# SimMarkt/RL_PtG

Measured on AMD Instinct MI355X. Metric: env-steps/sec at N=65536 envs; achieved HBM GB/s vs roofline, higher is better.
Workload: dtype f32 observations / rewards; env state, reward coefficients and cum_rew in f64

## Files before the change

### rl_ptg_amd/csrc/ptg_env.hip

```cpp
#include "ptg_handle.h"

#include <hip/hip_runtime.h>
#include <chrono>
#include <hip/hip_ext.h>

#include <algorithm>
#include <cmath>
#include <cstdarg>
#include <cstdio>
#include <cstdlib>
#include <cstring>
#include <string>
#include <type_traits>
#include <vector>

namespace {

constexpr int NT = PTG_N_TABLES;
constexpr int NC = PTG_N_COLS;
constexpr int N_DEST = 6;
constexpr int DEST_TID[N_DEST] = {PTG_T_COOLDOWN, PTG_T_STANDBY_UP, PTG_T_STANDBY_DOWN, PTG_T_STARTUP_COLD,
                                  PTG_T_STARTUP_HOT, PTG_T_OP1_START_P};

__device__ __forceinline__ int part_tid(int p) { return p == 0 ? PTG_T_OP1_START_P : 7 + p; }
// ... 2104 lines not shown
        if (std::chrono::steady_clock::now() - t0 > std::chrono::microseconds(200)) break;
    }
    HIP_TRY(h, hipStreamSynchronize(st));
    return 0;
}

int collect_error(ptg_env* h, hipStream_t st)
{
    const int rc = wait_stream(h, st);
    if (rc) return rc;
    return check_error_flags(h);
}

struct FinSpan { unsigned s0, n, c0, dropped; };
__device__ __forceinline__ FinSpan fin_span(unsigned total, unsigned ring_cap, unsigned cap, const unsigned* count, int append)
{
    FinSpan s;
    const unsigned have = total < ring_cap ? total : ring_cap;
    const unsigned held = append ? count[0] : 0u;
    s.c0 = held < cap ? held : cap;
    const unsigned room = cap - s.c0;
    s.n = have < room ? have : room;
    s.s0 = (total - have) % ring_cap;
    s.dropped = total - s.n;
    return s;
}

__global__ void __launch_bounds__(256)
k_fin_drain(const double* __restrict__ r_ret, const int* __restrict__ r_len, const int* __restrict__ r_env, const unsigned* __restrict__ r_count,
            unsigned ring_cap, double* __restrict__ ret, int* __restrict__ len, int* __restrict__ env, unsigned cap,
            const unsigned* __restrict__ count, int append, int env_offset)
{
    const FinSpan s = fin_span(*r_count, ring_cap, cap, count, append);
    for (unsigned i = blockIdx.x * 256u + threadIdx.x; i < s.n; i += gridDim.x * 256u) {
        unsigned slot = s.s0 + i;
        if (slot >= ring_cap) slot -= ring_cap;
        if (ret) ret[s.c0 + i] = r_ret[slot];
        if (len) len[s.c0 + i] = r_len[slot];
        if (env) env[s.c0 + i] = r_env[slot] + env_offset;
    }
}

__global__ void __launch_bounds__(64)
k_fin_commit(unsigned* r_count, unsigned ring_cap, unsigned cap, unsigned* count, int append)
{
    if (threadIdx.x != 0) return;
    const FinSpan s = fin_span(*r_count, ring_cap, cap, count, append);
    const unsigned before = append ? count[1] : 0u;
    count[0] = s.c0 + s.n;
    count[1] = before + s.dropped;
    *r_count = 0u;
}

__global__ void __launch_bounds__(1024)
k_fin_stats(const double* __restrict__ ret, const int* __restrict__ len, const unsigned* __restrict__ count, double* __restrict__ stats,
            int accumulate)
{
    __shared__ double part[16][5];
    const unsigned n = count[0];
    double s = 0.0, s2 = 0.0, sl = 0.0, mn = INFINITY, mx = -INFINITY;
#pragma unroll 4
    for (unsigned i = threadIdx.x; i < n; i += 1024u) {
        const double r = ret[i];
        s += r; s2 += r * r;
        if (len) sl += (double)len[i];
        mn = r < mn ? r : mn; mx = r > mx ? r : mx;
    }
    for (int off = 32; off > 0; off >>= 1) {
        s += __shfl_down(s, off); s2 += __shfl_down(s2, off); sl += __shfl_down(sl, off);
        const double a = __shfl_down(mn, off), b = __shfl_down(mx, off);
        mn = a < mn ? a : mn; mx = b > mx ? b : mx;
    }
    const int wave = threadIdx.x >> 6;
    if ((threadIdx.x & 63) == 0) { part[wave][0] = s; part[wave][1] = s2; part[wave][2] = sl; part[wave][3] = mn; part[wave][4] = mx; }
    __syncthreads();
    if (threadIdx.x != 0) return;
    for (int w = 1; w < 16; w++) {
        s += part[w][0]; s2 += part[w][1]; sl += part[w][2];
        mn = part[w][3] < mn ? part[w][3] : mn; mx = part[w][4] > mx ? part[w][4] : mx;
    }
    double c = (double)n;
    if (accumulate) {
        c += stats[0]; s += stats[1]; s2 += stats[2]; sl += stats[3];
        mn = stats[4] < mn ? stats[4] : mn; mx = stats[5] > mx ? stats[5] : mx;
    }
    stats[0] = c; stats[1] = s; stats[2] = s2; stats[3] = sl; stats[4] = mn; stats[5] = mx;
}

}

extern "C" {

int ptg_abi_version(void) { return PTG_ABI_VERSION; }

const char* ptg_last_error(const ptg_env* env) { return env ? env->err.c_str() : g_create_err.c_str(); }

int ptg_num_envs(const ptg_env* env) { return env ? env->n : PTG_E_INVALID; }
int ptg_obs_dim(const ptg_env* env) { return env ? env->F : PTG_E_INVALID; }

void ptg_destroy(ptg_env* env)
{
    if (!env) return;
    (void)hipSetDevice(env->device);
    (void)hipDeviceSynchronize();
    if (env->ref_stream) (void)hipStreamDestroy(env->ref_stream);
    if (env->ev_fork) (void)hipEventDestroy(env->ev_fork);
    if (env->ev_tail) (void)hipEventDestroy(env->ev_tail);
    for (void* p : env->allocs) (void)hipFree(p);
    if (env->d_tape) (void)hipFree(env->d_tape);
    if (env->d_eps_ind) (void)hipFree(env->d_eps_ind);
    if (env->vn_partials) (void)hipFree(env->vn_partials);
    if (env->vn_den) (void)hipFree(env->vn_den);
    if (env->vn_moments) (void)hipFree(env->vn_moments);
    if (env->err_host) (void)hipHostFree(env->err_host);
    if (env->fin_stage) (void)hipHostFree(env->fin_stage);
    for (void* q : {env->hs_act, env->hs_out, env->hs_final, (void*)env->hs_info}) if (q) (void)hipFree(q);
    for (auto& r : env->prof_used)
        for (hipEvent_t e : {r.e0, r.e1, r.h0, r.h1}) if (e) (void)hipEventDestroy(e);
    for (auto& p : env->prof_free) { (void)hipEventDestroy(p.first); (void)hipEventDestroy(p.second); }
    delete env;
}

int ptg_create(const ptg_config* cfg, const ptg_tables* tables, const ptg_market* sets, int n_sets, int n_envs,
               int device_id, ptg_env** out)
{
    if (!cfg || !tables || !sets || !out) return set_err(nullptr, PTG_E_INVALID, "ptg_create: null argument");
    if (n_envs <= 0 || n_sets < 1 || n_sets > PTG_MAX_MARKET_SETS) return set_err(nullptr, PTG_E_INVALID, "ptg_create: bad n_envs / n_sets");
    if (cfg->time_step_op <= 0 || cfg->sim_step <= 0 || cfg->price_ahead < 1 || cfg->price_ahead > 64)
        return set_err(nullptr, PTG_E_INVALID, "ptg_create: bad sim_step / time_step_op / price_ahead");
    if (cfg->out_dtype != PTG_OUT_F32 && cfg->out_dtype != PTG_OUT_F64) return set_err(nullptr, PTG_E_INVALID, "ptg_create: bad out_dtype");
    if (cfg->obs_layout < PTG_OBS_ROW_MAJOR || cfg->obs_layout > PTG_OBS_SPLIT) return set_err(nullptr, PTG_E_INVALID, "ptg_create: bad obs_layout");
    if (cfg->eps_sim_steps < 7) return set_err(nullptr, PTG_E_INVALID, "ptg_create: eps_sim_steps must be >= 7");
    int ndev = 0;
    hipError_t he = hipGetDeviceCount(&ndev);
    if (he != hipSuccess || ndev <= 0)
        return set_err(nullptr, PTG_E_HIP, "no HIP device available (%s): libptg_env has no CPU path", hipGetErrorString(he));
    if (device_id < 0 || device_id >= ndev) return set_err(nullptr, PTG_E_INVALID, "device %d out of range (%d devices)", device_id, ndev);
    he = hipSetDevice(device_id);
    if (he != hipSuccess) return set_err(nullptr, PTG_E_HIP, "hipSetDevice failed: %s", hipGetErrorString(he));

    ptg_env* h = new ptg_env();
    h->cfg = *cfg; h->n = n_envs; h->device = device_id; h->n_sets = n_sets;
    h->knob_no_hot = getenv("PTG_NO_HOT_KERNELS") != nullptr; h->knob_no_lds_lut = getenv("PTG_NO_LDS_LUT") != nullptr;
    h->knob_no_refresh = getenv("PTG_NO_REFRESH") != nullptr; h->knob_refresh_always = getenv("PTG_REFRESH_ALWAYS") != nullptr;
    {
        hipDeviceProp_t prop;
        if (hipGetDeviceProperties(&prop, device_id) == hipSuccess && prop.multiProcessorCount > 0) h->n_cu = prop.multiProcessorCount;
        else (void)hipGetLastError();
    }
    if (const char* v = getenv("PTG_PC_CHUNK")) h->knob_chunk = atoi(v);
    if (const char* v = getenv("PTG_BLOCK")) { const int b = atoi(v); if (b == 128 || b == 256 || b == 512) h->knob_block = b; }
    h->S = (int)((double)cfg->sim_step / (double)cfg->time_step_op);
    h->F = cfg->raw_modified ? 2 * cfg->price_ahead + 9 : cfg->price_ahead + 4 + 9;
    h->fast = (cfg->out_dtype == PTG_OUT_F32);
    h->fm = (cfg->obs_layout == PTG_OBS_FEATURE_MAJOR);
    memset(&h->P, 0, sizeof h->P);
    DevParams& P = h->P;
    int rc = 0;
    auto fail = [&](int code) { g_create_err = h->err; ptg_destroy(h); return code; };
    if (h->S < 1) { set_err(h, PTG_E_INVALID, "step_size < 1"); return fail(PTG_E_INVALID); }
// ... 72 lines not shown
        float2* d_sc32;
        if ((rc = dev_upload(h, &d_sc32, sc32.data(), sc32.size()))) return fail(rc);
        P.sincos32 = d_sc32;
        std::vector<float>& pool = h->pool32_host;
        h->off_sc = (unsigned)pool.size();
        for (size_t q = 0; q < sc32.size(); q++) { pool.push_back(sc32[q].x); pool.push_back(sc32[q].y); }
        pool.resize(pool.size() + 16, 0.f);
        float* d_pool;
        if ((rc = dev_upload(h, &d_pool, pool.data(), pool.size()))) return fail(rc);
        h->d_pool32 = d_pool;
        P.featA32 = d_pool; P.featB32 = d_pool + h->off_featB; P.gas_n32 = d_pool + h->off_gasn; P.eua_n32 = d_pool + h->off_euan;
        pool.clear(); pool.shrink_to_fit();
        std::vector<double>& p64 = h->pool64_host;
        h->o64_sc = (unsigned)p64.size();
        for (size_t q = 0; q < sc.size(); q++) { p64.push_back(sc[q].x); p64.push_back(sc[q].y); }
        p64.resize(p64.size() + 16, 0.0);
        double* d_p64;
        if ((rc = dev_upload(h, &d_p64, p64.data(), p64.size()))) return fail(rc);
        h->d_pool64 = d_p64;
        p64.clear(); p64.shrink_to_fit();
    }
    {
        const double f = P.sim_step_d / 3600;
        P.k_chp = cfg->convert_mol_to_Nm3 * cfg->H_u_CH4 * 1000 * (cfg->eta_CHP * cfg->eeg_el_price + (1 - cfg->eta_CHP) * cfg->heat_price) * f;
        P.k_eua = cfg->Molar_mass_CO2 / 1000 / 1000 * 3600 * 100 * f;
        RecFast* d_recf;
        if ((rc = dev_alloc(h, &d_recf, h->rec_total))) return fail(rc);
        hipLaunchKernelGGL(k_build_fast, dim3(grid_for((long long)h->rec_total, 256)), dim3(256), 0, 0, P, P.rec, d_recf, (int)h->rec_total);
        if ((rc = launch_check(h, "k_build_fast"))) return fail(rc);
        P.recf = d_recf;
        if ((rc = dev_alloc(h, &h->d_rkey, h->rec_total + 8))) return fail(rc);
        hipLaunchKernelGGL(k_extract_keys, dim3(grid_for((long long)h->rec_total, 256)), dim3(256), 0, 0, d_recf, h->d_rkey, (int)h->rec_total);
        if ((rc = launch_check(h, "k_extract_keys"))) return fail(rc);
    }

    if ((rc = dev_alloc(h, &P.st_a, n_envs)) || (rc = dev_alloc(h, &P.st_b, n_envs)) || (rc = dev_alloc(h, &P.st_c, n_envs)))
        return fail(rc);
    P.fin_cap = std::max(2 * n_envs, 1024);
    if ((rc = dev_alloc(h, &P.fin_ret, P.fin_cap)) || (rc = dev_alloc(h, &P.fin_len, P.fin_cap)) ||
        (rc = dev_alloc(h, &P.fin_env, P.fin_cap)) || (rc = dev_alloc(h, &P.fin_count, 1)))
        return fail(rc);
    {
        void* dp = nullptr;
        if (hipHostMalloc((void**)&h->err_host, 6 * sizeof(int), hipHostMallocMapped) != hipSuccess ||
            hipHostGetDevicePointer(&dp, h->err_host, 0) != hipSuccess) { set_err(h, PTG_E_HIP, "hipHostMalloc of the error words failed"); return fail(PTG_E_HIP); }
        h->err_host[0] = 0; h->err_host[1] = 0; h->err_host[2] = 0; h->err_host[3] = 0; h->err_host[4] = 0; h->err_host[5] = 0;
        P.err = (int*)dp;
    }
    if ((rc = dev_alloc(h, &P.term_flag, 4))) return fail(rc);
    if (hipMemset(P.term_flag, 0, 4 * sizeof(int)) != hipSuccess) { set_err(h, PTG_E_HIP, "hipMemset failed"); return fail(PTG_E_HIP); }
    h->d_desync = P.term_flag + 1;
    if ((rc = set_desync(h, nullptr, true, true))) return fail(rc);
    {
        const size_t need = (size_t)P.fin_cap * (sizeof(double) + 2 * sizeof(int));
        if (hipHostMalloc(&h->fin_stage, need, hipHostMallocDefault) == hipSuccess) h->fin_stage_bytes = need;
        else { (void)hipGetLastError(); h->fin_stage = nullptr; }
    }
    if (hipMemset(P.fin_count, 0, sizeof(int)) != hipSuccess) {
        set_err(h, PTG_E_HIP, "hipMemset failed");
        return fail(PTG_E_HIP);
    }
    {
        const int lad[LAD_N] = {P.t1_start_p_f, P.t2_start_f_p, P.t_p_f, P.t_f_p, P.t1_p_f_p, P.t2_p_f_p, P.t3_p_f_p, P.t34_p_f_p, P.t4_p_f_p,
                                P.t45_p_f_p, P.t5_p_f_p, P.t1_f_p_f, P.t2_f_p_f, P.t23_f_p_f, P.t3_f_p_f, P.t34_f_p_f, P.t4_f_p_f, P.t45_f_p_f,
                                P.t5_f_p_f, P.i_full, P.j_full};
        if ((rc = dev_upload(h, &h->d_ladder, lad, LAD_N))) return fail(rc);
    }
    hipLaunchKernelGGL(k_init_state, dim3(grid_for(n_envs, 256)), dim3(256), 0, 0, P, 0, 0);
    if ((rc = launch_check(h, "k_init_state"))) return fail(rc);
    if (!h->knob_no_refresh) {
        int lo = 0, hi = 0;
        (void)hipDeviceGetStreamPriorityRange(&lo, &hi);
        if (hipStreamCreateWithPriority(&h->ref_stream, hipStreamNonBlocking, hi) != hipSuccess) { h->ref_stream = nullptr; (void)hipGetLastError(); }
        if (hipEventCreateWithFlags(&h->ev_fork, hipEventDisableTiming) != hipSuccess) {
            (void)hipGetLastError();
            if (h->ref_stream) { (void)hipStreamDestroy(h->ref_stream); h->ref_stream = nullptr; }
        }
    }
    if (hipDeviceSynchronize() != hipSuccess) { set_err(h, PTG_E_HIP, "device synchronize failed after init"); return fail(PTG_E_HIP); }
    *out = h;
    return 0;
}

int ptg_set_market_assignment(ptg_env* h, const uint8_t* set_of_env_host)
{
    if (!h || !set_of_env_host) return set_err(h, PTG_E_INVALID, "null argument");
    HIP_TRY(h, hipSetDevice(h->device));
    HIP_TRY(h, hipDeviceSynchronize());
    std::vector<StA> a(h->n);
    HIP_TRY(h, hipMemcpy(a.data(), h->P.st_a, sizeof(StA) * h->n, hipMemcpyDeviceToHost));
    for (int e = 0; e < h->n; e++) {
        if (set_of_env_host[e] >= h->n_sets) return set_err(h, PTG_E_INVALID, "env %d: market set %d out of range", e, set_of_env_host[e]);
        a[e].flags = (a[e].flags & ~(3u << 15)) | ((unsigned)set_of_env_host[e] << 15);
    }
    HIP_TRY(h, hipMemcpy(h->P.st_a, a.data(), sizeof(StA) * h->n, hipMemcpyHostToDevice));
    return 0;
}

int ptg_set_episode_plan(ptg_env* h, const double* eps_ind_host, int n, int64_t first_ptr, int64_t stride)
{
    if (!h || n < 0 || (n > 0 && !eps_ind_host) || first_ptr < 0 || stride < 0) return set_err(h, PTG_E_INVALID, "bad episode plan");
    HIP_TRY(h, hipSetDevice(h->device));
    if (h->d_eps_ind) { (void)hipFree(h->d_eps_ind); h->d_eps_ind = nullptr; }
    h->P.E = n; h->P.eps_ind = nullptr; h->P.ep_stride = 0;
    if (n > 0) {
        std::vector<int> ei(n);
        for (int q = 0; q < n; q++) ei[q] = (int)eps_ind_host[q];
        HIP_TRY(h, hipMalloc((void**)&h->d_eps_ind, sizeof(int) * n));
        HIP_TRY(h, hipMemcpy(h->d_eps_ind, ei.data(), sizeof(int) * n, hipMemcpyHostToDevice));
        h->P.eps_ind = h->d_eps_ind;
        h->P.ep_stride = (int)(stride % n);
    }
    hipLaunchKernelGGL(k_init_state, dim3(grid_for(h->n, 256)), dim3(256), 0, 0, h->P, n > 0 ? (int)(first_ptr % n) : 0, 1);
    int rc = launch_check(h, "k_init_state");
// ... 83 lines not shown
    return 0;
}

int ptg_set_global_env_offset(ptg_env* h, int64_t offset)
{
    if (!h || offset < 0) return set_err(h, PTG_E_INVALID, "bad env offset");
    h->P.env_offset = (long long)offset;
    return 0;
}

int ptg_get_noise_tape(ptg_env* h, double* tape_host)
{
    if (!h || !tape_host) return set_err(h, PTG_E_INVALID, "null argument");
    if (h->tape_len <= 0) return set_err(h, PTG_E_INVALID, "no noise tape set");
    HIP_TRY(h, hipSetDevice(h->device));
    HIP_TRY(h, hipDeviceSynchronize());
    double* tmp = nullptr;
    const size_t bytes = sizeof(double) * (size_t)h->n * h->tape_len;
    HIP_TRY(h, hipMalloc((void**)&tmp, bytes));
    hipLaunchKernelGGL(k_transpose, dim3((h->n + 31) / 32, (h->tape_len + 31) / 32), dim3(32, 8), 0, 0, (const double*)h->d_tape, tmp, h->tape_len, h->n);
    hipError_t e = hipDeviceSynchronize();
    if (e == hipSuccess) e = hipMemcpy(tape_host, tmp, bytes, hipMemcpyDeviceToHost);
    (void)hipFree(tmp);
    if (e != hipSuccess) return set_err(h, PTG_E_HIP, "noise tape download failed: %s", hipGetErrorString(e));
    return 0;
}

int ptg_reset(ptg_env* h, const uint8_t* mask_host, void* obs_dev, void* stream)
{
    if (!h) return PTG_E_INVALID;
    HIP_TRY(h, hipSetDevice(h->device));
    hipStream_t st = as_stream(stream);
    uint8_t* d_mask = nullptr;
    if (mask_host) {
        HIP_TRY(h, hipMalloc((void**)&d_mask, h->n));
        HIP_TRY(h, hipMemcpyAsync(d_mask, mask_host, h->n, hipMemcpyHostToDevice, st));
    }
    const dim3 grid(grid_for(h->n, 256)), block(256);
    if (h->cfg.out_dtype == PTG_OUT_F64) {
        if (h->fm) hipLaunchKernelGGL((k_reset<double, false, true, 0>), grid, block, 0, st, h->P, d_mask, (double*)obs_dev);
        else hipLaunchKernelGGL((k_reset<double, false, false, 0>), grid, block, 0, st, h->P, d_mask, (double*)obs_dev);
    } else {
        if (h->fm) hipLaunchKernelGGL((k_reset<float, true, true, 0>), grid, block, 0, st, h->P, d_mask, (float*)obs_dev);
        else hipLaunchKernelGGL((k_reset<float, true, false, 0>), grid, block, 0, st, h->P, d_mask, (float*)obs_dev);
    }
    int rc = launch_check(h, "k_reset");
    if (d_mask) { (void)hipStreamSynchronize(st); (void)hipFree(d_mask); }
    if (rc) return rc;
    bool all = !mask_host;
    if (mask_host) { all = true; for (int e = 0; e < h->n && all; e++) all = mask_host[e] != 0; }
    if (all) { h->reset_done = true; h->sync_k = 0; }
    else h->sync_k = -1;
    return set_desync(h, st, !all);
}

static int launch_step_generic(ptg_env* h, hipStream_t st, const void* actions_dev, int action_kind, void* obs_dev, void* rew_dev,
                               uint8_t* done_dev, void* final_obs_dev, double* info_dev, int only_at_k = -1)
{
    const dim3 grid(grid_for(h->n, 256)), block(256);
    const bool f64 = h->cfg.out_dtype == PTG_OUT_F64;
    h->fin_maybe = true;
#define PTG_LAUNCH_STEP_(OUT, FAST, INFO, FM, PAC)                                                                     \
    hipLaunchKernelGGL((k_step<OUT, FAST, INFO, FM, PAC>), grid, block, 0, st, h->P, actions_dev, action_kind, (OUT*)obs_dev, \
                       (OUT*)rew_dev, done_dev, (OUT*)final_obs_dev, info_dev, only_at_k)
#define PTG_LAUNCH_STEP(OUT, FAST, INFO, FM)                                                                          \
    do { if (h->cfg.price_ahead == 13) PTG_LAUNCH_STEP_(OUT, FAST, INFO, FM, 13); else PTG_LAUNCH_STEP_(OUT, FAST, INFO, FM, 0); } while (0)
    if (f64) {
        if (info_dev) { if (h->fm) PTG_LAUNCH_STEP(double, false, true, true); else PTG_LAUNCH_STEP(double, false, true, false); }
        else { if (h->fm) PTG_LAUNCH_STEP(double, false, false, true); else PTG_LAUNCH_STEP(double, false, false, false); }
    } else if (info_dev) {
        if (h->fm) PTG_LAUNCH_STEP(float, false, true, true); else PTG_LAUNCH_STEP(float, false, true, false);
    } else {
        if (h->fm) PTG_LAUNCH_STEP(float, true, false, true); else PTG_LAUNCH_STEP(float, true, false, false);
    }
#undef PTG_LAUNCH_STEP
#undef PTG_LAUNCH_STEP_
    return launch_check(h, "k_step");
}

static int launch_rollout_generic(ptg_env* h, hipStream_t st, const void* actions_dev, int action_kind, int n_steps, void* obs_dev,
                                  void* rew_dev, uint8_t* done_dev, double* info_dev = nullptr)
{
    const size_t asz = action_kind == PTG_ACT_I64 ? 8 : 4, osz = h->cfg.out_dtype == PTG_OUT_F64 ? 8 : 4;
    for (int t = 0; t < n_steps; t++) {
        const int rc = launch_step_generic(h, st, (const char*)actions_dev + (size_t)t * h->n * asz, action_kind,
                                           (char*)obs_dev + (size_t)t * obs_step_elems(h) * osz, (char*)rew_dev + (size_t)t * h->n * osz,
                                           done_dev + (size_t)t * h->n, nullptr, info_dev ? info_dev + (size_t)t * h->n * PTG_N_INFO : nullptr);
        if (rc) return rc;
    }
    return 0;
}

int ptg_step(ptg_env* h, const void* actions_dev, int action_kind, void* obs_dev, void* rew_dev, uint8_t* done_dev,
             void* final_obs_dev, double* info_dev, void* stream)
{
    if (!h) return PTG_E_INVALID;
    if (!actions_dev || !obs_dev || !rew_dev || !done_dev) return set_err(h, PTG_E_INVALID, "ptg_step: null buffer");
    if (action_kind < PTG_ACT_I32 || action_kind > PTG_ACT_I64) return set_err(h, PTG_E_INVALID, "ptg_step: bad action_kind");
    if ((h->cfg.action_type == 1) != (action_kind == PTG_ACT_F32))
        return set_err(h, PTG_E_INVALID, "ptg_step: action_kind does not match cfg.action_type");
    if (!h->reset_done) return set_err(h, PTG_E_INVALID, "ptg_step: envs must be reset first");
    HIP_TRY(h, hipSetDevice(h->device));
    hipStream_t st = as_stream(stream);
    const int k_term = h->cfg.eps_sim_steps - 6;
    if (hot_eligible(h) && !info_dev && h->sync_k != k_term) {
        hipStreamCaptureStatus cs = hipStreamCaptureStatusNone;
        if (hipStreamIsCapturing(st, &cs) != hipSuccess) { (void)hipGetLastError(); cs = hipStreamCaptureStatusNone; }
        const bool capturing = cs != hipStreamCaptureStatusNone && h->replay_proof;
        h->step_skip_term = capturing ? 1 : 0;
        PTG_HOT_DISPATCH(launch_step_hot, h, st, actions_dev, action_kind, PTG_NOARG, obs_dev, rew_dev, done_dev);
        h->step_skip_term = 0;
        int rc = launch_check(h, "k_step_hot");
        if (!rc && capturing) rc = launch_step_generic(h, st, actions_dev, action_kind, obs_dev, rew_dev, done_dev, final_obs_dev, nullptr, k_term);
        h->sync_k += 1;
        return rc;
    }
    const int rc = launch_step_generic(h, st, actions_dev, action_kind, obs_dev, rew_dev, done_dev, final_obs_dev, info_dev);
    if (h->sync_k >= 0) h->sync_k = (h->sync_k == k_term) ? 0 : h->sync_k + 1;
    return rc;
}

static int rollout_impl(ptg_env* h, const char* what, const void* actions_dev, int action_kind, int n_steps, void* obs_dev, void* rew_dev,
                        uint8_t* done_dev, double* info_dev, void* stream)
{
    if (!h) return PTG_E_INVALID;
    if (!actions_dev || !obs_dev || !rew_dev || !done_dev || n_steps < 1) return set_err(h, PTG_E_INVALID, "%s: bad argument", what);
    if (action_kind < PTG_ACT_I32 || action_kind > PTG_ACT_I64) return set_err(h, PTG_E_INVALID, "%s: bad action_kind", what);
    if ((h->cfg.action_type == 1) != (action_kind == PTG_ACT_F32))
        return set_err(h, PTG_E_INVALID, "%s: action_kind does not match cfg.action_type", what);
    if (!h->reset_done) return set_err(h, PTG_E_INVALID, "%s: envs must be reset first", what);
// ... 18 lines not shown
            rc = launch_check(h, "k_rollout_pc");
            h->sync_k += cnt;
        } else if (h->sync_k >= 0) {
            cnt = 1;
            rc = launch_rollout_generic(h, st, a_t, action_kind, 1, o_t, r_t, d_t, i_t);
            h->sync_k = (h->sync_k == k_term) ? 0 : h->sync_k + 1;
        } else {
            cnt = n_steps - t0;
            rc = launch_rollout_generic(h, st, a_t, action_kind, cnt, o_t, r_t, d_t, i_t);
        }
        if (rc) return rc;
        t0 += cnt;
    }
    return 0;
}

int ptg_rollout(ptg_env* h, const void* actions_dev, int action_kind, int n_steps, void* obs_dev, void* rew_dev,
                uint8_t* done_dev, void* stream)
{
    return rollout_impl(h, "ptg_rollout", actions_dev, action_kind, n_steps, obs_dev, rew_dev, done_dev, nullptr, stream);
}

int ptg_rollout_info(ptg_env* h, const void* actions_dev, int action_kind, int n_steps, void* obs_dev, void* rew_dev,
                     uint8_t* done_dev, double* info_dev, void* stream)
{
    if (h && !info_dev) return set_err(h, PTG_E_INVALID, "ptg_rollout_info: bad argument");
    return rollout_impl(h, "ptg_rollout_info", actions_dev, action_kind, n_steps, obs_dev, rew_dev, done_dev, info_dev, stream);
}

int ptg_rollout_launches(ptg_env* h, int n_steps)
{
    if (!h || n_steps < 1) return PTG_E_INVALID;
    const int k_term = h->cfg.eps_sim_steps - 6;
    int k = h->sync_k, t0 = 0, launches = 0;
    while (t0 < n_steps) {
        if (hot_eligible(h) && k >= 0 && k != k_term) {
            const PcPlan pl = pc_plan(h);
            const int cnt = std::min(n_steps - t0, k_term - k);
            launches += ((cnt + pl.t_cap - 1) / pl.t_cap) * ((h->n + pl.chunk - 1) / pl.chunk);
            k += cnt; t0 += cnt;
        } else if (k >= 0) {
            launches += 1; k = (k == k_term) ? 0 : k + 1; t0 += 1;
        } else {
            launches += n_steps - t0; t0 = n_steps;
        }
    }
    return launches;
}

int ptg_note_replays(ptg_env* h, int n_steps)
{
    if (!h || n_steps < 0) return set_err(h, PTG_E_INVALID, "ptg_note_replays: bad argument");
    h->fin_maybe = true;
    if (h->sync_k < 0) return 0;
    const long long period = (long long)(h->cfg.eps_sim_steps - 6) + 1;
    h->sync_k = (int)(((long long)h->sync_k + n_steps) % period);
    return 0;
}

int ptg_set_replay_proof(ptg_env* h, int enable)
{
    if (!h) return PTG_E_INVALID;
    h->replay_proof = enable ? 1 : 0;
    return 0;
}

int ptg_steps_to_episode_end(ptg_env* h, int* steps)
{
    if (!h || !steps) return set_err(h, PTG_E_INVALID, "bad argument");
    *steps = h->sync_k >= 0 ? (h->cfg.eps_sim_steps - 6) - h->sync_k + 1 : 0;
    return 0;
}

int ptg_host_layout_ex(const ptg_env* h, size_t* off_rew, size_t* off_done, size_t* off_status, size_t* total)
{
    if (!h) return PTG_E_INVALID;
    const size_t osz = h->cfg.out_dtype == PTG_OUT_F64 ? 8 : 4;
    const size_t o_rew = (obs_step_elems(h) * osz + 15) / 16 * 16, o_done = (o_rew + (size_t)h->n * osz + 15) / 16 * 16;
    const size_t o_status = (o_done + (size_t)h->n + 15) / 16 * 16;
    if (off_rew) *off_rew = o_rew;
    if (off_done) *off_done = o_done;
    if (off_status) *off_status = o_status;
    if (total) *total = (o_status + (size_t)h->n + 15) / 16 * 16;
    return 0;
}

int ptg_host_layout(const ptg_env* h, size_t* off_rew, size_t* off_done, size_t* total) { return ptg_host_layout_ex(h, off_rew, off_done, nullptr, total); }

namespace {

void status_column(const ptg_env* h, int& c0, int& onehot)
{
    const int q_stat = h->cfg.raw_modified ? 2 * h->cfg.price_ahead : h->cfg.price_ahead + 4;
    onehot = (h->flat || h->split) ? 1 : 0;
    c0 = h->split ? 0 : q_stat;
    if (h->flat) c0 = h->status_col_flat;
}

int wait_event(ptg_env* h, hipEvent_t ev)
{
    const auto t0 = std::chrono::steady_clock::now();
    for (;;) {
        const hipError_t q = hipEventQuery(ev);
        if (q == hipSuccess) return 0;
        if (q != hipErrorNotReady) return set_err(h, PTG_E_HIP, "hipEventQuery failed: %s", hipGetErrorString(q));
        (void)hipGetLastError();
// ... 271 lines not shown
        switch (field) {
        case PTG_F_I: a[e].i = ii[e]; break;
        case PTG_F_J: a[e].j = ii[e]; break;
        case PTG_F_K: a[e].k = ii[e]; break;
        case PTG_F_ACT_EP_D: b[e].act_d = ii[e]; break;
        case PTG_F_EP_PTR:
            if (ii[e] < 0 || (P.E > 0 && ii[e] >= P.E)) return set_err(h, PTG_E_INVALID, "episode pointer out of range");
            c[e].epp = ii[e]; break;
        case PTG_F_NOISE_COUNT: b[e].nctr = ii[e]; break;
        case PTG_F_N_STATE_CHANGES: c[e].nchg = ii[e]; break;
        case PTG_F_CUM_REW: b[e].cum = id[e]; break;
        case PTG_F_METH_STATE: if (ii[e] < 0 || ii[e] > 4) return set_err(h, PTG_E_INVALID, "bad meth_state"); f = put(f, 0, 7, ii[e]); break;
        case PTG_F_HOT_COLD: f = put(f, 3, 1, ii[e] != 0); break;
        case PTG_F_STANDBY_TID: f = put(f, 4, 1, ii[e] == PTG_T_STANDBY_UP); break;
        case PTG_F_STARTUP_TID: f = put(f, 5, 1, ii[e] == PTG_T_STARTUP_HOT); break;
        case PTG_F_PARTIAL_TID: {
            int t = ii[e];
            if (t != PTG_T_OP1_START_P && (t < PTG_T_OP4_P_F_P_5 || t > PTG_T_OP8_F_P)) return set_err(h, PTG_E_INVALID, "bad partial table id");
            f = put(f, 6, 7, t == PTG_T_OP1_START_P ? 0 : t - 7); break;
        }
        case PTG_F_FULL_TID: {
            int t = ii[e];
            if (t != PTG_T_OP2_START_F && t != PTG_T_OP3_P_F && (t < PTG_T_OP9_F_P_F_5 || t > PTG_T_OP12_F_P_F_20)) return set_err(h, PTG_E_INVALID, "bad full table id");
            f = put(f, 9, 7, t == PTG_T_OP2_START_F ? 0 : (t == PTG_T_OP3_P_F ? 1 : t - 11)); break;
        }
        case PTG_F_CURRENT_ACTION: if (ii[e] < 0 || ii[e] > 4) return set_err(h, PTG_E_INVALID, "bad action"); f = put(f, 12, 7, ii[e]); break;
        case PTG_F_MARKET_SET: if (ii[e] < 0 || ii[e] >= h->n_sets) return set_err(h, PTG_E_INVALID, "bad market set"); f = put(f, 15, 3, ii[e]); break;
        case PTG_F_T_CAT: {
            auto it = std::lower_bound(h->Tvals.begin(), h->Tvals.end(), id[e]);
            if (it == h->Tvals.end() || *it != id[e]) return set_err(h, PTG_E_INVALID, "T_cat %.17g of env %d is not a table temperature", id[e], e);
            f = (f & 0x1FFFFu) | ((unsigned)(it - h->Tvals.begin()) << 17); break;
        }
        default: return set_err(h, PTG_E_INVALID, "unknown state field %d", field);
        }
        a[e].flags = f;
    }
    HIP_TRY(h, hipMemcpy(P.st_a, a.data(), sizeof(StA) * n, hipMemcpyHostToDevice));
    HIP_TRY(h, hipMemcpy(P.st_b, b.data(), sizeof(StB) * n, hipMemcpyHostToDevice));
    HIP_TRY(h, hipMemcpy(P.st_c, c.data(), sizeof(StC) * n, hipMemcpyHostToDevice));
    if (field == PTG_F_K) {
        bool same = true;
        for (int e = 1; e < n; e++) same = same && (a[e].k == a[0].k);
        h->sync_k = (same && a[0].k >= 0 && a[0].k <= h->cfg.eps_sim_steps - 6) ? a[0].k : -1;
        return set_desync(h, nullptr, h->sync_k < 0, true);
    }
    return 0;
}

int ptg_finished_episodes(ptg_env* h, double* returns_host, int32_t* lengths_host, int32_t* env_ids_host, int cap, int* count)
{
    if (!h || !count || cap < 0) return set_err(h, PTG_E_INVALID, "bad argument");
    if (!h->fin_maybe) { *count = 0; return 0; }
    HIP_TRY(h, hipSetDevice(h->device));
    HIP_TRY(h, hipDeviceSynchronize());
    h->fin_maybe = false;
    unsigned total = 0;
    HIP_TRY(h, hipMemcpy(&total, h->P.fin_count, sizeof(unsigned), hipMemcpyDeviceToHost));
    const int have = (int)std::min<unsigned>(total, (unsigned)h->P.fin_cap);
    const int n = std::min(have, cap);
    h->fin_dropped += (unsigned long long)(total - (unsigned)have) + (unsigned long long)(have - n);
    if (n > 0) {
        const int cap_r = h->P.fin_cap, s0 = (int)((total - (unsigned)have) % (unsigned)cap_r);
        const int n0 = std::min(n, cap_r - s0), n1 = n - n0;
        const size_t need = (size_t)n * (sizeof(double) + 2 * sizeof(int));
        if (need > h->fin_stage_bytes) {
            if (h->fin_stage) (void)hipHostFree(h->fin_stage);
            h->fin_stage = nullptr; h->fin_stage_bytes = 0;
            if (hipHostMalloc(&h->fin_stage, need, hipHostMallocDefault) != hipSuccess) { (void)hipGetLastError(); h->fin_stage = nullptr; }
            else h->fin_stage_bytes = need;
        }
        char* stage = (char*)h->fin_stage;
        double* s_ret = stage ? (double*)stage : returns_host;
        int* s_len = stage ? (int*)(stage + (size_t)n * sizeof(double)) : lengths_host;
        int* s_env = stage ? s_len + n : env_ids_host;
        auto pull = [&](void* dst, const void* src0, const void* src_wrap, size_t el) -> hipError_t {
            if (!dst) return hipSuccess;
            hipError_t e = hipMemcpyAsync(dst, src0, el * n0, hipMemcpyDeviceToHost, nullptr);
            if (e == hipSuccess && n1) e = hipMemcpyAsync((char*)dst + el * n0, src_wrap, el * n1, hipMemcpyDeviceToHost, nullptr);
            return e;
        };
        if (returns_host) HIP_TRY(h, pull(s_ret, h->P.fin_ret + s0, h->P.fin_ret, sizeof(double)));
        if (lengths_host) HIP_TRY(h, pull(s_len, h->P.fin_len + s0, h->P.fin_len, sizeof(int)));
        if (env_ids_host) HIP_TRY(h, pull(s_env, h->P.fin_env + s0, h->P.fin_env, sizeof(int)));
        HIP_TRY(h, hipStreamSynchronize(nullptr));
        if (stage) {
            if (returns_host) memcpy(returns_host, s_ret, sizeof(double) * n);
            if (lengths_host) memcpy(lengths_host, s_len, sizeof(int) * n);
            if (env_ids_host) memcpy(env_ids_host, s_env, sizeof(int) * n);
        }
    }
    HIP_TRY(h, hipMemset(h->P.fin_count, 0, sizeof(int)));
    *count = n;
    return 0;
}

int ptg_finished_dropped(ptg_env* h, uint64_t* dropped_total)
{
    if (!h || !dropped_total) return set_err(h, PTG_E_INVALID, "bad argument");
    *dropped_total = h->fin_dropped;
    return 0;
}

int ptg_finished_episodes_dev(ptg_env* h, double* ret_dev, int32_t* len_dev, int32_t* env_dev, int cap, uint32_t* count_dev, int append,
                              void* stream)
{
    if (!h || !count_dev || cap < 1 || (!ret_dev && !len_dev && !env_dev)) return set_err(h, PTG_E_INVALID, "ptg_finished_episodes_dev: bad argument");
    HIP_TRY(h, hipSetDevice(h->device));
    const DevParams& P = h->P;
    hipStream_t st = as_stream(stream);
    const int blocks = std::min(grid_for(std::min(cap, P.fin_cap), 256), 1024);
    hipLaunchKernelGGL(k_fin_drain, dim3((unsigned)blocks), dim3(256), 0, st, (const double*)P.fin_ret, (const int*)P.fin_len, (const int*)P.fin_env,
                       (const unsigned*)P.fin_count, (unsigned)P.fin_cap, ret_dev, len_dev, env_dev, (unsigned)cap, (const unsigned*)count_dev,
                       append ? 1 : 0, (int)P.env_offset);
    int rc = launch_check(h, "k_fin_drain");
    if (rc) return rc;
    hipLaunchKernelGGL(k_fin_commit, dim3(1), dim3(64), 0, st, (unsigned*)P.fin_count, (unsigned)P.fin_cap, (unsigned)cap, count_dev, append ? 1 : 0);
    return launch_check(h, "k_fin_commit");
}

int ptg_episode_stats_dev(ptg_env* h, const double* ret_dev, const int32_t* len_dev, const uint32_t* count_dev, double* stats_dev,
                          int accumulate, void* stream)
{
    if (!h || !ret_dev || !count_dev || !stats_dev) return set_err(h, PTG_E_INVALID, "ptg_episode_stats_dev: bad argument");
    HIP_TRY(h, hipSetDevice(h->device));
    hipLaunchKernelGGL(k_fin_stats, dim3(1), dim3(1024), 0, as_stream(stream), ret_dev, len_dev, count_dev, stats_dev, accumulate ? 1 : 0);
    return launch_check(h, "k_fin_stats");
}

int ptg_market_feature_series(ptg_env* h, int which, float* out_host, int cap, int* count)
{
    if (!h || !count || which < 0 || which > 3 || cap < 0) return set_err(h, PTG_E_INVALID, "ptg_market_feature_series: bad argument");
    HIP_TRY(h, hipSetDevice(h->device));
    const bool hourly = which < 2;
    const int n = h->n_sets * (hourly ? h->P.n_hours : h->P.n_days);
    const unsigned off = which == 0 ? 0u : which == 1 ? h->off_featB : which == 2 ? h->off_gasn : h->off_euan;
    *count = n;
    if (out_host) {
        if (cap < n) return set_err(h, PTG_E_INVALID, "ptg_market_feature_series: buffer too small (%d < %d)", cap, n);
        HIP_TRY(h, hipMemcpy(out_host, h->d_pool32 + off, sizeof(float) * n, hipMemcpyDeviceToHost));
    }
    return 0;
}

#ifdef PTG_STAMPS
int ptg_debug_stamps(unsigned long long* out_host) { return (int)hipMemcpyFromSymbol(out_host, HIP_SYMBOL(g_stamps), sizeof(g_stamps)); }
// ... 39 lines not shown
```

### rl_ptg_amd/csrc/ptg_handle.h

```cpp
#ifndef PTG_HANDLE_H
#define PTG_HANDLE_H

#include "../../include/ptg_env.h"

#include <hip/hip_runtime.h>

#include <algorithm>
#include <string>
#include <utility>
#include <vector>

namespace {

struct alignas(64) Rec {
    double T;
    double m[5];
    int tkey;
    int pad;
    double spare;
};
static_assert(sizeof(Rec) == 64, "Rec must be 64 bytes");

struct alignas(64) RecFast {
    double base, ch4, c_gas, c_el;
// ... 35 lines not shown
    const int* argidx;
    const double* Tvals;
    const double* tape;
    const int* eps_ind;
    const double2* sincos;
    const float2* sincos32;
    const double *el, *featA, *featB, *gas, *eua, *gas_n, *eua_n;
    const float *featA32, *featB32, *gas_n32, *eua_n32;
    const double *pot_raw, *pf_raw;
    const double2* setc;
    StA* st_a; StB* st_b; StC* st_c;
    double* fin_ret; int* fin_len; int* fin_env; int* fin_count; int fin_cap;
    const int* cmap; int q_stat;
    int split;
    int* err;
    int* term_flag;
};

__device__ __forceinline__ unsigned lowbias32(unsigned x)
{
    x ^= x >> 16; x *= 0x7feb352du; x ^= x >> 15; x *= 0x846ca68bu; x ^= x >> 16;
    return x;
}

}

struct ptg_env {
    ptg_config cfg;
    int n = 0, device = 0, n_sets = 0, F = 0, S = 0;
    bool reset_done = false;
    DevParams P;
    std::vector<void*> allocs;
    std::vector<double> Tvals;
    std::vector<int> tab_rows, rec_base;
    size_t rec_total = 0;
    bool fast = false, fm = false, flat = false, split = false;
    double* d_tape = nullptr;
    unsigned short* d_lut16 = nullptr;
    unsigned short* d_rkey = nullptr;
    float* d_pool32 = nullptr; double* d_pool64 = nullptr;
    unsigned off_featB = 0, off_gasn = 0, off_euan = 0, off_gas = 0, off_eua = 0, off_sc = 0;
    unsigned o64_featA = 0, o64_featB = 0, o64_gasn = 0, o64_euan = 0, o64_sc = 0;
    std::vector<float> pool32_host;
    std::vector<double> pool64_host;
    int* d_ladder = nullptr;
    int sync_k = -1;
    int step_skip_term = 0;
    int replay_proof = 0;
    double *vn_returns = nullptr, *vn_stats = nullptr, *vn_partials = nullptr, *vn_den = nullptr, *vn_moments = nullptr;
    size_t vn_partials_cap = 0; int vn_T_cap = 0;
    double vn_gamma = 0.99, vn_eps = 1e-8, vn_clip = 10.0;
    bool fin_maybe = false;
    void* fin_stage = nullptr; size_t fin_stage_bytes = 0;
    unsigned long long fin_dropped = 0;
    int tape_len = 0;
    double *d_pot_raw = nullptr, *d_pf_raw = nullptr;
    int* d_eps_ind = nullptr;
    bool knob_no_hot = false, knob_no_lds_lut = false, knob_no_refresh = false, knob_refresh_always = false;
    int front_horizon = 0;
    hipStream_t ref_stream = nullptr;
    hipEvent_t ev_fork = nullptr;
    double unrefreshed_bytes = 1e18;
    int n_cu = 256;
    std::vector<const void*> attr_done;
    int* err_host = nullptr;
    int* d_desync = nullptr;
    void *hs_act = nullptr, *hs_out = nullptr, *hs_final = nullptr; double* hs_info = nullptr;
    struct HostStep {
        bool active = false, zc = false, tail_done = false;
        void* out_host = nullptr; void* final_host = nullptr; double* info_host = nullptr;
        hipStream_t st = nullptr;
        int n_done = 0;
    } hs;
    int status_col_flat = 5;
    hipEvent_t ev_tail = nullptr;
    struct HostPtr { const void* host = nullptr; void* dev = nullptr; };
    HostPtr hs_map[8]; int hs_next = 0;
    int knob_chunk = 65536, knob_block = 0;
    double* rollout_info = nullptr;
    bool profiling = false;
    struct ProfRec { hipEvent_t e0 = nullptr, e1 = nullptr, h0 = nullptr, h1 = nullptr; };
    std::vector<ProfRec> prof_used;
    std::vector<std::pair<hipEvent_t, hipEvent_t>> prof_free;
    std::string err;
};

__attribute__((visibility("hidden"))) int set_err(ptg_env* h, int code, const char* fmt, ...);

namespace {

#define HIP_TRY(h, call)                                                                              \
    do {                                                                                              \
        hipError_t e_ = (call);                                                                       \
        if (e_ != hipSuccess) return set_err(h, PTG_E_HIP, "%s failed: %s", #call, hipGetErrorString(e_)); \
    } while (0)

template <typename T>
int dev_alloc(ptg_env* h, T** p, size_t count)
{
    void* q = nullptr;
    HIP_TRY(h, hipMalloc(&q, std::max<size_t>(count, 1) * sizeof(T)));
    h->allocs.push_back(q);
    *p = (T*)q;
    return 0;
}

// ... 15 lines not shown
```

Baseline: 36.01 billion.

## Drain finished episodes via GPU kernel into mapped host block, event-gated

Replaces the finished-episode readback, which used a count memcpy, several async memcpys, a staging copy and a memset, with a drain kernel plus commit kernel that write straight into a zero-copy mapped host block with a header. It also records an event at the episode-finishing step so the drain can wait on that event instead of only on a full device sync. The aim is fewer host round trips and API calls on the episode-collection path. In exchange it adds event-state tracking that must be invalidated on capture, replays and stream changes. It also makes host allocation failure a hard error, and the event path still ends with a device synchronize.

New measurement: 35.46 billion. -1.5%, worse.

```diff
diff --git a/rl_ptg_amd/csrc/ptg_env.hip b/rl_ptg_amd/csrc/ptg_env.hip
--- a/rl_ptg_amd/csrc/ptg_env.hip
+++ b/rl_ptg_amd/csrc/ptg_env.hip
@@ -2180,6 +2180,24 @@
     *r_count = 0u;
 }
 
+int fin_drain_to_block(ptg_env* h, bool want_ret, bool want_len, bool want_env, int cap)
+{
+    const DevParams& P = h->P;
+    char* blk = h->fin_stage_dev;
+    const size_t ring = (size_t)P.fin_cap;
+    const unsigned k_cap = (unsigned)std::min(cap, P.fin_cap);
+    unsigned* hdr = (unsigned*)blk;
+    const int blocks = std::max(1, std::min(grid_for((long long)k_cap, 256), 1024));
+    hipLaunchKernelGGL(k_fin_drain, dim3((unsigned)blocks), dim3(256), 0, nullptr, (const double*)P.fin_ret, (const int*)P.fin_len, (const int*)P.fin_env,
+                       (const unsigned*)P.fin_count, (unsigned)P.fin_cap, want_ret ? (double*)(blk + 16) : nullptr,
+                       want_len ? (int*)(blk + 16 + 8 * ring) : nullptr, want_env ? (int*)(blk + 16 + 12 * ring) : nullptr, k_cap,
+                       (const unsigned*)hdr, 0, 0);
+    const int rc = launch_check(h, "k_fin_drain");
+    if (rc) return rc;
+    hipLaunchKernelGGL(k_fin_commit, dim3(1), dim3(64), 0, nullptr, (unsigned*)P.fin_count, (unsigned)P.fin_cap, k_cap, hdr, 0);
+    return launch_check(h, "k_fin_commit");
+}
+
 __global__ void __launch_bounds__(1024)
 k_fin_stats(const double* __restrict__ ret, const int* __restrict__ len, const unsigned* __restrict__ count, double* __restrict__ stats,
             int accumulate)
@@ -2234,6 +2252,7 @@
     if (env->ref_stream) (void)hipStreamDestroy(env->ref_stream);
     if (env->ev_fork) (void)hipEventDestroy(env->ev_fork);
     if (env->ev_tail) (void)hipEventDestroy(env->ev_tail);
+    if (env->ev_fin) (void)hipEventDestroy(env->ev_fin);
     for (void* p : env->allocs) (void)hipFree(p);
     if (env->d_tape) (void)hipFree(env->d_tape);
     if (env->d_eps_ind) (void)hipFree(env->d_eps_ind);
@@ -2412,14 +2431,20 @@
     h->d_desync = P.term_flag + 1;
     if ((rc = set_desync(h, nullptr, true, true))) return fail(rc);
     {
-        const size_t need = (size_t)P.fin_cap * (sizeof(double) + 2 * sizeof(int));
-        if (hipHostMalloc(&h->fin_stage, need, hipHostMallocDefault) == hipSuccess) h->fin_stage_bytes = need;
-        else { (void)hipGetLastError(); h->fin_stage = nullptr; }
+        const size_t need = 16 + (size_t)P.fin_cap * (sizeof(double) + 2 * sizeof(int));
+        void* dp = nullptr;
+        if (hipHostMalloc(&h->fin_stage, need, hipHostMallocMapped) != hipSuccess ||
+            hipHostGetDevicePointer(&dp, h->fin_stage, 0) != hipSuccess) { set_err(h, PTG_E_HIP, "hipHostMalloc of the finished-episode block failed"); return fail(PTG_E_HIP); }
+        h->fin_stage_bytes = need;
+        h->fin_stage_dev = (char*)dp;
+        memset(h->fin_stage, 0, need);
     }
     if (hipMemset(P.fin_count, 0, sizeof(int)) != hipSuccess) {
         set_err(h, PTG_E_HIP, "hipMemset failed");
         return fail(PTG_E_HIP);
     }
+    if ((rc = fin_drain_to_block(h, true, true, true, P.fin_cap))) return fail(rc);
+    if (hipEventCreateWithFlags(&h->ev_fin, hipEventDisableTiming) != hipSuccess) { (void)hipGetLastError(); h->ev_fin = nullptr; }
     {
         const int lad[LAD_N] = {P.t1_start_p_f, P.t2_start_f_p, P.t_p_f, P.t_f_p, P.t1_p_f_p, P.t2_p_f_p, P.t3_p_f_p, P.t34_p_f_p, P.t4_p_f_p,
                                 P.t45_p_f_p, P.t5_p_f_p, P.t1_f_p_f, P.t2_f_p_f, P.t23_f_p_f, P.t3_f_p_f, P.t34_f_p_f, P.t4_f_p_f, P.t45_f_p_f,
@@ -2609,6 +2634,20 @@
     if (all) { h->reset_done = true; h->sync_k = 0; }
     else h->sync_k = -1;
     return set_desync(h, st, !all);
+}
+
+static int note_finishing_launch(ptg_env* h, hipStream_t st)
+{
+    if (h->fin_ev_state == ptg_env::FIN_EV_UNKNOWN) return 0;
+    if (h->sync_k < 0 || !h->ev_fin) { h->fin_ev_state = ptg_env::FIN_EV_UNKNOWN; return 0; }
+    hipStreamCaptureStatus cs = hipStreamCaptureStatusNone;
+    if (hipStreamIsCapturing(st, &cs) != hipSuccess) { (void)hipGetLastError(); cs = hipStreamCaptureStatusActive; }
+    if (cs != hipStreamCaptureStatusNone) { h->fin_ev_state = ptg_env::FIN_EV_UNKNOWN; return 0; }
+    if (h->sync_k != h->cfg.eps_sim_steps - 6) return 0;
+    if (h->fin_ev_state == ptg_env::FIN_EV_ONE && st != h->fin_ev_stream) { h->fin_ev_state = ptg_env::FIN_EV_UNKNOWN; return 0; }
+    if (hipEventRecord(h->ev_fin, st) != hipSuccess) { (void)hipGetLastError(); h->fin_ev_state = ptg_env::FIN_EV_UNKNOWN; return 0; }
+    h->fin_ev_state = ptg_env::FIN_EV_ONE; h->fin_ev_stream = st;
+    return 0;
 }
 
 static int launch_step_generic(ptg_env* h, hipStream_t st, const void* actions_dev, int action_kind, void* obs_dev, void* rew_dev,
@@ -2632,7 +2671,9 @@
     }
 #undef PTG_LAUNCH_STEP
 #undef PTG_LAUNCH_STEP_
-    return launch_check(h, "k_step");
+    const int rc = launch_check(h, "k_step");
+    if (rc) { h->fin_ev_state = ptg_env::FIN_EV_UNKNOWN; return rc; }
+    return note_finishing_launch(h, st);
 }
 
 static int launch_rollout_generic(ptg_env* h, hipStream_t st, const void* actions_dev, int action_kind, int n_steps, void* obs_dev,
@@ -2757,6 +2798,7 @@
 {
     if (!h || n_steps < 0) return set_err(h, PTG_E_INVALID, "ptg_note_replays: bad argument");
     h->fin_maybe = true;
+    h->fin_ev_state = ptg_env::FIN_EV_UNKNOWN;
     if (h->sync_k < 0) return 0;
     const long long period = (long long)(h->cfg.eps_sim_steps - 6) + 1;
     h->sync_k = (int)(((long long)h->sync_k + n_steps) % period);
@@ -3134,45 +3176,28 @@
     if (!h || !count || cap < 0) return set_err(h, PTG_E_INVALID, "bad argument");
     if (!h->fin_maybe) { *count = 0; return 0; }
     HIP_TRY(h, hipSetDevice(h->device));
-    HIP_TRY(h, hipDeviceSynchronize());
+    const bool by_event = h->fin_ev_state == ptg_env::FIN_EV_ONE;
+    h->fin_ev_state = ptg_env::FIN_EV_NONE;
     h->fin_maybe = false;
-    unsigned total = 0;
-    HIP_TRY(h, hipMemcpy(&total, h->P.fin_count, sizeof(unsigned), hipMemcpyDeviceToHost));
-    const int have = (int)std::min<unsigned>(total, (unsigned)h->P.fin_cap);
-    const int n = std::min(have, cap);
-    h->fin_dropped += (unsigned long long)(total - (unsigned)have) + (unsigned long long)(have - n);
-    if (n > 0) {
-        const int cap_r = h->P.fin_cap, s0 = (int)((total - (unsigned)have) % (unsigned)cap_r);
-        const int n0 = std::min(n, cap_r - s0), n1 = n - n0;
-        const size_t need = (size_t)n * (sizeof(double) + 2 * sizeof(int));
-        if (need > h->fin_stage_bytes) {
-            if (h->fin_stage) (void)hipHostFree(h->fin_stage);
-            h->fin_stage = nullptr; h->fin_stage_bytes = 0;
-            if (hipHostMalloc(&h->fin_stage, need, hipHostMallocDefault) != hipSuccess) { (void)hipGetLastError(); h->fin_stage = nullptr; }
-            else h->fin_stage_bytes = need;
-        }
-        char* stage = (char*)h->fin_stage;
-        double* s_ret = stage ? (double*)stage : returns_host;
-        int* s_len = stage ? (int*)(stage + (size_t)n * sizeof(double)) : lengths_host;
-        int* s_env = stage ? s_len + n : env_ids_host;
-        auto pull = [&](void* dst, const void* src0, const void* src_wrap, size_t el) -> hipError_t {
-            if (!dst) return hipSuccess;
-            hipError_t e = hipMemcpyAsync(dst, src0, el * n0, hipMemcpyDeviceToHost, nullptr);
-            if (e == hipSuccess && n1) e = hipMemcpyAsync((char*)dst + el * n0, src_wrap, el * n1, hipMemcpyDeviceToHost, nullptr);
-            return e;
-        };
-        if (returns_host) HIP_TRY(h, pull(s_ret, h->P.fin_ret + s0, h->P.fin_ret, sizeof(double)));
-        if (lengths_host) HIP_TRY(h, pull(s_len, h->P.fin_len + s0, h->P.fin_len, sizeof(int)));
-        if (env_ids_host) HIP_TRY(h, pull(s_env, h->P.fin_env + s0, h->P.fin_env, sizeof(int)));
-        HIP_TRY(h, hipStreamSynchronize(nullptr));
-        if (stage) {
-            if (returns_host) memcpy(returns_host, s_ret, sizeof(double) * n);
-            if (lengths_host) memcpy(lengths_host, s_len, sizeof(int) * n);
-            if (env_ids_host) memcpy(env_ids_host, s_env, sizeof(int) * n);
-        }
-    }
-    HIP_TRY(h, hipMemset(h->P.fin_count, 0, sizeof(int)));
-    *count = n;
+    int rc;
+    if (by_event) {
+        HIP_TRY(h, hipStreamWaitEvent(nullptr, h->ev_fin, 0));
+        if ((rc = fin_drain_to_block(h, returns_host != nullptr, lengths_host != nullptr, env_ids_host != nullptr, cap))) return rc;
+        if ((rc = wait_stream(h, nullptr))) return rc;
+        HIP_TRY(h, hipDeviceSynchronize());
+    } else {
+        HIP_TRY(h, hipDeviceSynchronize());
+        if ((rc = fin_drain_to_block(h, returns_host != nullptr, lengths_host != nullptr, env_ids_host != nullptr, cap))) return rc;
+        if ((rc = wait_stream(h, nullptr))) return rc;
+    }
+    const char* blk = (const char*)h->fin_stage;
+    const unsigned* hdr = (const unsigned*)blk;
+    const size_t n = hdr[0], ring = (size_t)h->P.fin_cap;
+    h->fin_dropped += hdr[1];
+    if (returns_host) memcpy(returns_host, blk + 16, sizeof(double) * n);
+    if (lengths_host) memcpy(lengths_host, blk + 16 + 8 * ring, sizeof(int) * n);
+    if (env_ids_host) memcpy(env_ids_host, blk + 16 + 12 * ring, sizeof(int) * n);
+    *count = (int)n;
     return 0;
 }
 
diff --git a/rl_ptg_amd/csrc/ptg_handle.h b/rl_ptg_amd/csrc/ptg_handle.h
--- a/rl_ptg_amd/csrc/ptg_handle.h
+++ b/rl_ptg_amd/csrc/ptg_handle.h
@@ -111,6 +111,10 @@
     double vn_gamma = 0.99, vn_eps = 1e-8, vn_clip = 10.0;
     bool fin_maybe = false;
     void* fin_stage = nullptr; size_t fin_stage_bytes = 0;
+    char* fin_stage_dev = nullptr;
+    enum { FIN_EV_NONE = 0, FIN_EV_ONE, FIN_EV_UNKNOWN };
+    int fin_ev_state = FIN_EV_NONE;
+    hipEvent_t ev_fin = nullptr; hipStream_t fin_ev_stream = nullptr;
     unsigned long long fin_dropped = 0;
     int tape_len = 0;
     double *d_pot_raw = nullptr, *d_pf_raw = nullptr;
```
